# pengfeidip/pytorch-faster-rcnn

Measured on AMD Instinct MI355X. Metric: img/s FasterRCNN_R50_FPN 1000x600 fwd+loss, higher is better.
Workload: dtype f32; 1 GPU; configs/faster_rcnn_r50_fpn.py (BASELINE config 2) forward_train; conv_algorithms=MIOpen benchmarked (warmup, at most 32 tuning iterations per solver), trunk=hipGraph replay (backbone + neck + RPN head convs), global_batch=2, imgs_per_gpu=2, image=600x1000 padded 608x1024, parallelism=dp1, sampler=device, mode=fwd

## Files before the change

pytorch-faster-rcnn_amd/csrc/conv3x3_wino_kernels.h:

```cpp
#pragma once
#include "common.h"

namespace frh {

typedef float wg_f32x16 __attribute__((ext_vector_type(16)));
typedef float wg_f32x2 __attribute__((ext_vector_type(2)));

constexpr int kWgThreads = 256;
constexpr int kWgBK = 8;
constexpr int kWgSide = 8;
constexpr int kWgCout = 64;
constexpr int kWgXcds = 8;
constexpr int kWgMaxLevels = 8;
constexpr int kWgSlab = 64 * kWgBK;
constexpr int kWgStage = 2 * 16 * kWgSlab;

struct Conv3x3Level {
  const float* x;
  const float* u;
  const float* bias;
  float* y;
  int64_t sn;
  int32_t sy, sx;
  int32_t h, w;
  int32_t by, bx;
  int32_t first;
};

struct Conv3x3Args {
  Conv3x3Level lv[kWgMaxLevels];
  int32_t levels, n, cin, cout, relu;
  int32_t total, chunk;
};

__device__ __forceinline__ int wg_slab_off(int r, int kh) { return r * kWgBK + ((kh ^ ((r >> 3) & 1)) << 2); }

struct Conv3x3Weights {
  const float* w[kWgMaxLevels];
  float* u[kWgMaxLevels];
};

__global__ void __launch_bounds__(256) conv3x3_bias_act_weights_kernel(const Conv3x3Weights tab, int cin, int cout) {
  const int64_t idx = (int64_t)blockIdx.x * 256 + threadIdx.x;
  if (idx >= (int64_t)(cin / kWgBK) * cout * 2) return;
  const float* w = tab.w[0];
  float* u = tab.u[0];
#pragma unroll
  for (int i = 1; i < kWgMaxLevels; ++i)
    if (i == (int)blockIdx.y) w = tab.w[i], u = tab.u[i];
  const int kh = (int)(idx & 1);
  const int co = (int)((idx >> 1) % cout);
  const int ch = (int)((idx >> 1) / cout);
  const float* wp = w + (int64_t)co * 9 * cin + ch * kWgBK + kh * 4;
  float g[3][3][4];
#pragma unroll
  for (int ky = 0; ky < 3; ++ky)
#pragma unroll
    for (int kx = 0; kx < 3; ++kx) {
      const float4 v = *reinterpret_cast<const float4*>(wp + (ky * 3 + kx) * cin);
      g[ky][kx][0] = v.x, g[ky][kx][1] = v.y, g[ky][kx][2] = v.z, g[ky][kx][3] = v.w;
    }
  float t[4][3][4];
#pragma unroll
  for (int kx = 0; kx < 3; ++kx)
#pragma unroll
    for (int c = 0; c < 4; ++c) {
      const float s = g[0][kx][c] + g[2][kx][c];
      t[0][kx][c] = g[0][kx][c];
      t[1][kx][c] = (s + g[1][kx][c]) * 0.5f;
      t[2][kx][c] = (s - g[1][kx][c]) * 0.5f;
      t[3][kx][c] = g[2][kx][c];
    }
  float* up = u + ((int64_t)ch * 16 * cout + co) * kWgBK + ((kh ^ ((co >> 3) & 1)) << 2);
#pragma unroll
  for (int a = 0; a < 4; ++a) {
    float o[4][4];
#pragma unroll
    for (int c = 0; c < 4; ++c) {
      const float s = t[a][0][c] + t[a][2][c];
      o[0][c] = t[a][0][c];
      o[1][c] = (s + t[a][1][c]) * 0.5f;
      o[2][c] = (s - t[a][1][c]) * 0.5f;
      o[3][c] = t[a][2][c];
    }
#pragma unroll
    for (int b = 0; b < 4; ++b)
      *reinterpret_cast<float4*>(up + (int64_t)(a * 4 + b) * cout * kWgBK) =
          make_float4(o[b][0], o[b][1], o[b][2], o[b][3]);
  }
}

__global__ void __launch_bounds__(kWgThreads) conv3x3_bias_act_wino_kernel(const Conv3x3Args a) {
  __shared__ __attribute__((aligned(16))) float lds[2 * kWgStage];

  const int wg = (int)(blockIdx.x % kWgXcds) * a.chunk + (int)(blockIdx.x / kWgXcds);
  if (wg >= a.total) return;
  Conv3x3Level L = a.lv[0];
#pragma unroll
  for (int i = 1; i < kWgMaxLevels; ++i)
    if (i < a.levels && wg >= a.lv[i].first) L = a.lv[i];
  const int H = L.h, W = L.w;
  int rest = wg - L.first;
  const int bx = rest % L.bx;
  rest /= L.bx;
  const int by = rest % L.by;
  rest /= L.by;
  const int img = rest % a.n;
  const int cb = rest / a.n;

  const int tid = threadIdx.x;
  const int lane = tid & 63, wave = tid >> 6;
  const int wm = wave >> 1, wn = wave & 1;
  const int h = lane >> 5, j = lane & 31;

  const int T = tid >> 2, c2 = tid & 3;
  const int iy0 = (by * kWgSide + (T >> 3)) * 2 - 1;
  const int ix0 = (bx * kWgSide + (T & 7)) * 2 - 1;
  const char* xb = reinterpret_cast<const char*>(L.x + (int64_t)img * L.sn);
  uint32_t xoff[4][4];
  bool xok[4][4];
#pragma unroll
  for (int r = 0; r < 4; ++r)
#pragma unroll
    for (int c = 0; c < 4; ++c) {
      const int iy = iy0 + r, ix = ix0 + c;
      xok[r][c] = iy >= 0 && iy < H && ix >= 0 && ix < W;
      const int cy = min(max(iy, 0), H - 1), cx = min(max(ix, 0), W - 1);
      xoff[r][c] = (uint32_t)(cy * L.sy + cx * L.sx + c2 * 2) * 4u;
    }
  const int v_off = wg_slab_off(T, c2 >> 1) + (c2 & 1) * 2;
  const char* ub = reinterpret_cast<const char*>(L.u + (int64_t)cb * kWgCout * kWgBK);
  const uint32_t u_src = (uint32_t)((tid >> 7) * a.cout * kWgBK + (tid & 127) * 4) * 4u;
  const int64_t u_pos = (int64_t)2 * a.cout * kWgBK * 4;
  const int64_t u_chunk = (int64_t)16 * a.cout * kWgBK * 4;
  const int u_off = 16 * kWgSlab + (tid >> 7) * kWgSlab + (tid & 127) * 4;
  const int a_off = wg_slab_off(wm * 32 + j, h);
  const int b_off = 16 * kWgSlab + wg_slab_off(wn * 32 + j, h);

  wg_f32x2 x00, x01, x02, x03, x10, x11, x12, x13, x20, x21, x22, x23, x30, x31, x32, x33;
  float4 u0, u1, u2, u3, u4, u5, u6, u7;
#define FRH_WG_LX(r, c) x##r##c = *reinterpret_cast<const wg_f32x2*>(xs_ + xoff[r][c])
#define FRH_WG_LU(q) *reinterpret_cast<const float4*>(up_ + (q) * u_pos + u_src)
#define FRH_WG_LOAD(t)                                                                   \
  do {                                                                                   \
    const char* xs_ = xb + (t) * (kWgBK * 4);                                               \
    FRH_WG_LX(0, 0), FRH_WG_LX(0, 1), FRH_WG_LX(0, 2), FRH_WG_LX(0, 3);                  \
    FRH_WG_LX(1, 0), FRH_WG_LX(1, 1), FRH_WG_LX(1, 2), FRH_WG_LX(1, 3);                  \
    FRH_WG_LX(2, 0), FRH_WG_LX(2, 1), FRH_WG_LX(2, 2), FRH_WG_LX(2, 3);                  \
    FRH_WG_LX(3, 0), FRH_WG_LX(3, 1), FRH_WG_LX(3, 2), FRH_WG_LX(3, 3);                  \
    const char* up_ = ub + (t) * u_chunk;                                                \
    u0 = FRH_WG_LU(0), u1 = FRH_WG_LU(1), u2 = FRH_WG_LU(2), u3 = FRH_WG_LU(3);          \
    u4 = FRH_WG_LU(4), u5 = FRH_WG_LU(5), u6 = FRH_WG_LU(6), u7 = FRH_WG_LU(7);          \
  } while (0)

#define FRH_WG_Z(r, c) (xok[r][c] ? x##r##c : z2)
#define FRH_WG_VROW(vp, e0, e1, e2, e3)                                   \
  do {                                                                    \
    *reinterpret_cast<wg_f32x2*>(vp) = (e0) - (e2);                       \
    *reinterpret_cast<wg_f32x2*>((vp) + kWgSlab) = (e1) + (e2);           \
    *reinterpret_cast<wg_f32x2*>((vp) + 2 * kWgSlab) = (e2) - (e1);       \
    *reinterpret_cast<wg_f32x2*>((vp) + 3 * kWgSlab) = (e1) - (e3);       \
  } while (0)
#define FRH_WG_STORE(ST)                                                                             \
  do {                                                                                               \
    float* sp = lds + (ST) * kWgStage;                                                               \
    float* uq = sp + u_off;                                                                          \
    *reinterpret_cast<float4*>(uq) = u0, *reinterpret_cast<float4*>(uq + 2 * kWgSlab) = u1;          \
    *reinterpret_cast<float4*>(uq + 4 * kWgSlab) = u2, *reinterpret_cast<float4*>(uq + 6 * kWgSlab) = u3;   \
    *reinterpret_cast<float4*>(uq + 8 * kWgSlab) = u4, *reinterpret_cast<float4*>(uq + 10 * kWgSlab) = u5;  \
    *reinterpret_cast<float4*>(uq + 12 * kWgSlab) = u6, *reinterpret_cast<float4*>(uq + 14 * kWgSlab) = u7; \
    const wg_f32x2 z2 = {0.0f, 0.0f};                                                                \
    const wg_f32x2 d00 = FRH_WG_Z(0, 0), d01 = FRH_WG_Z(0, 1), d02 = FRH_WG_Z(0, 2), d03 = FRH_WG_Z(0, 3); \
    const wg_f32x2 d10 = FRH_WG_Z(1, 0), d11 = FRH_WG_Z(1, 1), d12 = FRH_WG_Z(1, 2), d13 = FRH_WG_Z(1, 3); \
    const wg_f32x2 d20 = FRH_WG_Z(2, 0), d21 = FRH_WG_Z(2, 1), d22 = FRH_WG_Z(2, 2), d23 = FRH_WG_Z(2, 3); \
    const wg_f32x2 d30 = FRH_WG_Z(3, 0), d31 = FRH_WG_Z(3, 1), d32 = FRH_WG_Z(3, 2), d33 = FRH_WG_Z(3, 3); \
    float* vp = sp + v_off;                                                                          \
    FRH_WG_VROW(vp, d00 - d20, d01 - d21, d02 - d22, d03 - d23);                                     \
    FRH_WG_VROW(vp + 4 * kWgSlab, d10 + d20, d11 + d21, d12 + d22, d13 + d23);                       \
    FRH_WG_VROW(vp + 8 * kWgSlab, d20 - d10, d21 - d11, d22 - d12, d23 - d13);                       \
    FRH_WG_VROW(vp + 12 * kWgSlab, d10 - d30, d11 - d31, d12 - d32, d13 - d33);                      \
  } while (0)

#define FRH_WG_MFMA(ST, p)                                                          \
  do {                                                                              \
    const float* sp = lds + (ST) * kWgStage + (p) * kWgSlab;                        \
    const float4 av = *reinterpret_cast<const float4*>(sp + a_off);                 \
    const float4 bv = *reinterpret_cast<const float4*>(sp + b_off);                 \
    acc[p] = __builtin_amdgcn_mfma_f32_32x32x2f32(av.x, bv.x, acc[p], 0, 0, 0);     \
    acc[p] = __builtin_amdgcn_mfma_f32_32x32x2f32(av.y, bv.y, acc[p], 0, 0, 0);     \
    acc[p] = __builtin_amdgcn_mfma_f32_32x32x2f32(av.z, bv.z, acc[p], 0, 0, 0);     \
    acc[p] = __builtin_amdgcn_mfma_f32_32x32x2f32(av.w, bv.w, acc[p], 0, 0, 0);     \
  } while (0)

#define FRH_WG_GROUPS(N, MEM, ID)                                                     \
  _Pragma("unroll") for (int p = 0; p < (N); ++p) {                                 \
    __builtin_amdgcn_sched_group_barrier(0x100, 2, ID);                             \
    _Pragma("unroll") for (int m = 0; m < 4; ++m) {                                 \
      __builtin_amdgcn_sched_group_barrier(0x008, 1, ID);                           \
      __builtin_amdgcn_sched_group_barrier(0x002, 2, ID);                           \
      __builtin_amdgcn_sched_group_barrier(MEM, 1, ID);                             \
    }                                                                               \
  }
#define FRH_WG_STEP(ST, STORE, LOAD, t)                                             \
  do {                                                                              \
    _Pragma("unroll") for (int p = 0; p < 16; ++p) FRH_WG_MFMA(ST, p);              \
    if (STORE) FRH_WG_STORE((ST) ^ 1);                                              \
    if (LOAD) FRH_WG_LOAD((t) + 2);                                                 \
    if (STORE) {                                                                    \
      __builtin_amdgcn_sched_group_barrier(0x100, 4, ST);                           \
      FRH_WG_GROUPS(4, 0x200, ST);                                                     \
      FRH_WG_GROUPS(6, 0x020, ST);                                                     \
      FRH_WG_GROUPS(6, 0x200, ST);                                                     \
    }                                                                               \
    if (STORE) {                                                                    \
      __syncthreads();                                                              \
      __builtin_amdgcn_sched_barrier(0);                                            \
    }                                                                               \
  } while (0)

  wg_f32x16 acc[16];
#pragma unroll
  for (int p = 0; p < 16; ++p)
#pragma unroll
    for (int r = 0; r < 16; ++r) acc[p][r] = 0.0f;

  const int steps = a.cin / kWgBK;
  FRH_WG_LOAD(0);
  FRH_WG_STORE(0);
  if (steps > 1) FRH_WG_LOAD(1);
  __syncthreads();
  int t = 0;
  for (; t + 3 < steps; t += 2) {
    FRH_WG_STEP(0, true, true, t);
    FRH_WG_STEP(1, true, true, t + 1);
  }
  if (t + 3 == steps) {
    FRH_WG_STEP(0, true, true, t);
    FRH_WG_STEP(1, true, false, t + 1);
    FRH_WG_STEP(0, false, false, t + 2);
  } else if (t + 2 == steps) {
    FRH_WG_STEP(0, true, false, t);
    FRH_WG_STEP(1, false, false, t + 1);
  } else {
    FRH_WG_STEP(0, false, false, t);
  }
#undef FRH_WG_LX
#undef FRH_WG_LU
#undef FRH_WG_LOAD
#undef FRH_WG_Z
#undef FRH_WG_VROW
#undef FRH_WG_STORE
#undef FRH_WG_MFMA
#undef FRH_WG_GROUPS
#undef FRH_WG_STEP

  const int co = cb * kWgCout + wn * 32 + j;
  const bool has_bias = L.bias != nullptr;
  const float bias = has_bias ? L.bias[co] : 0.0f;
  float* yb = L.y + (int64_t)img * H * W * a.cout + co;
#pragma unroll
  for (int r = 0; r < 16; ++r) {
    const int oy = (by * kWgSide + wm * 4 + (r >> 2)) * 2;
    const int ox = (bx * kWgSide + (r & 3) + 4 * h) * 2;
    float s0[4], s1[4];
#pragma unroll
    for (int b = 0; b < 4; ++b) {
      s0[b] = (acc[b][r] + acc[4 + b][r]) + acc[8 + b][r];
      s1[b] = (acc[4 + b][r] - acc[8 + b][r]) - acc[12 + b][r];
    }
    float o[2][2];
    o[0][0] = (s0[0] + s0[1]) + s0[2];
    o[0][1] = (s0[1] - s0[2]) - s0[3];
    o[1][0] = (s1[0] + s1[1]) + s1[2];
    o[1][1] = (s1[1] - s1[2]) - s1[3];
#pragma unroll
    for (int dy = 0; dy < 2; ++dy)
#pragma unroll
      for (int dx = 0; dx < 2; ++dx) {
        float v = o[dy][dx];
        if (has_bias) v = v + bias;
        if (a.relu) v = fmaxf(v, 0.0f);
        if (oy + dy < H && ox + dx < W) yb[((int64_t)(oy + dy) * W + (ox + dx)) * a.cout] = v;
      }
  }
}

struct Conv3x3LevelDesc {
  const float* x;
  const float* wt;
  const float* bias;
  float* y;
  int32_t h, w;
  int64_t sn, sy, sx;
};

inline int32_t conv3x3_launch(const char* what, int32_t levels, const Conv3x3LevelDesc* d, float* ws,
                              int64_t ws_floats, int64_t n, int32_t cin, int32_t cout, int32_t relu, void* stream) {
  FRH_REQUIRE(levels >= 1 && levels <= kWgMaxLevels, "1 to %d levels, got %d", kWgMaxLevels, levels);
  FRH_REQUIRE(n >= 0 && n < (1 << 20) && cin >= 1 && cout >= 1 && cout <= (1 << 20), "bad sizes");
  FRH_REQUIRE(cin % kWgBK == 0 && cout % kWgCout == 0, "cin %d must be a multiple of %d and cout %d of %d", cin,
              kWgBK, cout, kWgCout);
  FRH_REQUIRE(ws, "null pointer argument");
  FRH_REQUIRE((uintptr_t)ws % 16 == 0, "tensors must be 16-byte aligned");
  const int64_t slot = (int64_t)16 * cin * cout;
  Conv3x3Weights tab = {};
  int slots = 0;
  Conv3x3Args a;
  a.levels = 0, a.n = (int32_t)n, a.cin = cin, a.cout = cout, a.relu = relu;
  int64_t total = 0;
  for (int i = 0; i < levels; ++i) {
    const Conv3x3LevelDesc& s = d[i];
    FRH_REQUIRE(s.h >= 0 && s.w >= 0, "bad sizes");
    if (n == 0 || s.h == 0 || s.w == 0) continue;
    FRH_REQUIRE(s.x && s.y && s.wt, "null pointer argument");
    FRH_REQUIRE(((uintptr_t)s.x | (uintptr_t)s.y | (uintptr_t)s.bias | (uintptr_t)s.wt) % 16 == 0,
                "tensors must be 16-byte aligned");
    if (slots == 0 || tab.w[slots - 1] != s.wt) {
      FRH_REQUIRE((slots + 1) * slot <= ws_floats, "workspace holds %lld floats, %d weights need %lld",
                  (long long)ws_floats, slots + 1, (long long)((slots + 1) * slot));
      tab.w[slots] = s.wt, tab.u[slots] = ws + slots * slot;
      ++slots;
    }
    FRH_REQUIRE(s.sn >= 0 && s.sy >= 0 && s.sx >= cin && (s.sn | s.sy | s.sx) % 4 == 0,
                "x strides must be multiples of 4 elements and the column stride at least cin");
    const int64_t span = (int64_t)(s.h - 1) * s.sy + (int64_t)(s.w - 1) * s.sx + cin;
    FRH_REQUIRE(span < ((int64_t)1 << 30), "one image of x spans too many elements");
    const int64_t x_end = (n - 1) * s.sn + span, y_end = n * s.h * s.w * cout;
    FRH_REQUIRE(s.y + y_end <= s.x || s.x + x_end <= s.y, "y must not alias x");
    FRH_REQUIRE(s.y + y_end <= ws || ws + ws_floats <= s.y, "y must not alias the workspace");
    Conv3x3Level& L = a.lv[a.levels++];
    L.x = s.x, L.u = tab.u[slots - 1], L.bias = s.bias, L.y = s.y;
    L.sn = s.sn, L.sy = (int32_t)s.sy, L.sx = (int32_t)s.sx, L.h = s.h, L.w = s.w;
    L.by = (s.h + 2 * kWgSide - 1) / (2 * kWgSide), L.bx = (s.w + 2 * kWgSide - 1) / (2 * kWgSide);
    L.first = (int32_t)total;
    total += (int64_t)L.by * L.bx * n * (cout / kWgCout);
    FRH_REQUIRE(total < ((int64_t)1 << 30), "too many blocks");
  }
  if (a.levels == 0) return FRH_OK;
  a.total = (int32_t)total;
  a.chunk = (int32_t)((total + kWgXcds - 1) / kWgXcds);
  const int64_t wt = (int64_t)(cin / kWgBK) * cout * 2;
  hipLaunchKernelGGL(conv3x3_bias_act_weights_kernel, dim3((unsigned)((wt + 255) / 256), (unsigned)slots), dim3(256),
                     0, as_stream(stream), tab, cin, cout);
  hipLaunchKernelGGL(conv3x3_bias_act_wino_kernel, dim3((unsigned)(a.chunk * kWgXcds)), dim3(kWgThreads), 0,
                     as_stream(stream), a);
  return check_launch(what);
}

}
```

Before: 376.0 img/s.

## Stream Winograd filter tiles via direct global-to-LDS loads and buffer loads

The Winograd 3x3 conv kernel now copies filter tiles straight from global memory into LDS with global_load_lds_dwordx4 through inline asm, instead of loading them into registers and storing them to LDS. Input tiles are read with raw buffer loads, which makes out-of-range reads safe, and are double-buffered in registers two steps ahead. The main loop is simplified to clamped step indices, with a combined waitcnt and barrier and a retuned schedule-group interleave. This is meant to cut VGPR pressure and VALU/LDS-store work in the main loop. In exchange it relies on hand-written m0 handling in inline asm and does redundant loads on the final steps.

```diff
diff --git a/pytorch-faster-rcnn_amd/csrc/conv3x3_wino_kernels.h b/pytorch-faster-rcnn_amd/csrc/conv3x3_wino_kernels.h
--- a/pytorch-faster-rcnn_amd/csrc/conv3x3_wino_kernels.h
+++ b/pytorch-faster-rcnn_amd/csrc/conv3x3_wino_kernels.h
@@ -13,7 +13,10 @@
 constexpr int kWgXcds = 8;
 constexpr int kWgMaxLevels = 8;
 constexpr int kWgSlab = 64 * kWgBK;
-constexpr int kWgStage = 2 * 16 * kWgSlab;
+constexpr int kWgImage = 16 * kWgSlab;
+
+typedef uint32_t wg_u32x2 __attribute__((ext_vector_type(2)));
+typedef __attribute__((address_space(3))) void* wg_lds_ptr;
 
 struct Conv3x3Level {
   const float* x;
@@ -90,8 +93,22 @@
   }
 }
 
+__device__ __forceinline__ __amdgpu_buffer_rsrc_t wg_buffer(const void* p) {
+  const uint64_t v = reinterpret_cast<uint64_t>(p);
+  const uint32_t lo = __builtin_amdgcn_readfirstlane((uint32_t)v);
+  const uint32_t hi = __builtin_amdgcn_readfirstlane((uint32_t)(v >> 32));
+  return __builtin_amdgcn_make_buffer_rsrc(reinterpret_cast<void*>(((uint64_t)hi << 32) | lo), 0, -1, 0x00020000);
+}
+
+__device__ __forceinline__ uint64_t wg_uniform64(const void* p) {
+  const uint64_t v = reinterpret_cast<uint64_t>(p);
+  const uint32_t lo = __builtin_amdgcn_readfirstlane((uint32_t)v);
+  const uint32_t hi = __builtin_amdgcn_readfirstlane((uint32_t)(v >> 32));
+  return ((uint64_t)hi << 32) | lo;
+}
+
 __global__ void __launch_bounds__(kWgThreads) conv3x3_bias_act_wino_kernel(const Conv3x3Args a) {
-  __shared__ __attribute__((aligned(16))) float lds[2 * kWgStage];
+  __shared__ __attribute__((aligned(16))) float lds[4 * kWgImage];
 
   const int wg = (int)(blockIdx.x % kWgXcds) * a.chunk + (int)(blockIdx.x / kWgXcds);
   if (wg >= a.total) return;
@@ -109,14 +126,14 @@
   const int cb = rest / a.n;
 
   const int tid = threadIdx.x;
-  const int lane = tid & 63, wave = tid >> 6;
+  const int lane = tid & 63, wave = __builtin_amdgcn_readfirstlane(tid >> 6);
   const int wm = wave >> 1, wn = wave & 1;
   const int h = lane >> 5, j = lane & 31;
 
   const int T = tid >> 2, c2 = tid & 3;
   const int iy0 = (by * kWgSide + (T >> 3)) * 2 - 1;
   const int ix0 = (bx * kWgSide + (T & 7)) * 2 - 1;
-  const char* xb = reinterpret_cast<const char*>(L.x + (int64_t)img * L.sn);
+  const __amdgpu_buffer_rsrc_t xb = wg_buffer(L.x + (int64_t)img * L.sn);
   uint32_t xoff[4][4];
   bool xok[4][4];
 #pragma unroll
@@ -129,31 +146,51 @@
       xoff[r][c] = (uint32_t)(cy * L.sy + cx * L.sx + c2 * 2) * 4u;
     }
   const int v_off = wg_slab_off(T, c2 >> 1) + (c2 & 1) * 2;
-  const char* ub = reinterpret_cast<const char*>(L.u + (int64_t)cb * kWgCout * kWgBK);
-  const uint32_t u_src = (uint32_t)((tid >> 7) * a.cout * kWgBK + (tid & 127) * 4) * 4u;
-  const int64_t u_pos = (int64_t)2 * a.cout * kWgBK * 4;
-  const int64_t u_chunk = (int64_t)16 * a.cout * kWgBK * 4;
-  const int u_off = 16 * kWgSlab + (tid >> 7) * kWgSlab + (tid & 127) * 4;
-  const int a_off = wg_slab_off(wm * 32 + j, h);
-  const int b_off = 16 * kWgSlab + wg_slab_off(wn * 32 + j, h);
-
-  wg_f32x2 x00, x01, x02, x03, x10, x11, x12, x13, x20, x21, x22, x23, x30, x31, x32, x33;
-  float4 u0, u1, u2, u3, u4, u5, u6, u7;
-#define FRH_WG_LX(r, c) x##r##c = *reinterpret_cast<const wg_f32x2*>(xs_ + xoff[r][c])
-#define FRH_WG_LU(q) *reinterpret_cast<const float4*>(up_ + (q) * u_pos + u_src)
-#define FRH_WG_LOAD(t)                                                                   \
-  do {                                                                                   \
-    const char* xs_ = xb + (t) * (kWgBK * 4);                                               \
-    FRH_WG_LX(0, 0), FRH_WG_LX(0, 1), FRH_WG_LX(0, 2), FRH_WG_LX(0, 3);                  \
-    FRH_WG_LX(1, 0), FRH_WG_LX(1, 1), FRH_WG_LX(1, 2), FRH_WG_LX(1, 3);                  \
-    FRH_WG_LX(2, 0), FRH_WG_LX(2, 1), FRH_WG_LX(2, 2), FRH_WG_LX(2, 3);                  \
-    FRH_WG_LX(3, 0), FRH_WG_LX(3, 1), FRH_WG_LX(3, 2), FRH_WG_LX(3, 3);                  \
-    const char* up_ = ub + (t) * u_chunk;                                                \
-    u0 = FRH_WG_LU(0), u1 = FRH_WG_LU(1), u2 = FRH_WG_LU(2), u3 = FRH_WG_LU(3);          \
-    u4 = FRH_WG_LU(4), u5 = FRH_WG_LU(5), u6 = FRH_WG_LU(6), u7 = FRH_WG_LU(7);          \
-  } while (0)
-
-#define FRH_WG_Z(r, c) (xok[r][c] ? x##r##c : z2)
+  const int64_t u_pos = (int64_t)a.cout * kWgBK * 4;
+  const int64_t u_chunk = 16 * u_pos;
+  const char* ub = reinterpret_cast<const char*>(L.u + (int64_t)cb * kWgCout * kWgBK) + wave * 4 * u_pos;
+  const uint32_t u_lane = (uint32_t)lane * 16u;
+  const uint32_t u_dst = (uint32_t)(uintptr_t)(wg_lds_ptr)lds + (uint32_t)wave * 4 * kWgSlab * 4;
+  const int a_off = 2 * kWgImage + wg_slab_off(wm * 32 + j, h);
+  const int b_off = wg_slab_off(wn * 32 + j, h);
+
+  wg_f32x2 x000, x001, x002, x003, x010, x011, x012, x013, x020, x021, x022, x023, x030, x031, x032, x033;
+  wg_f32x2 x100, x101, x102, x103, x110, x111, x112, x113, x120, x121, x122, x123, x130, x131, x132, x133;
+  const wg_f32x2 z2 = {0.0f, 0.0f};
+#define FRH_WG_LX(S, r, c) \
+  x##S##r##c = __builtin_bit_cast(wg_f32x2, __builtin_amdgcn_raw_buffer_load_b64(xb, (int)xoff[r][c], xs_, 0))
+#define FRH_WG_LOADX(S, t)                                                                       \
+  do {                                                                                           \
+    const int xs_ = (t) * (kWgBK * 4);                                                           \
+    FRH_WG_LX(S, 0, 0), FRH_WG_LX(S, 0, 1), FRH_WG_LX(S, 0, 2), FRH_WG_LX(S, 0, 3);              \
+    FRH_WG_LX(S, 1, 0), FRH_WG_LX(S, 1, 1), FRH_WG_LX(S, 1, 2), FRH_WG_LX(S, 1, 3);              \
+    FRH_WG_LX(S, 2, 0), FRH_WG_LX(S, 2, 1), FRH_WG_LX(S, 2, 2), FRH_WG_LX(S, 2, 3);              \
+    FRH_WG_LX(S, 3, 0), FRH_WG_LX(S, 3, 1), FRH_WG_LX(S, 3, 2), FRH_WG_LX(S, 3, 3);              \
+  } while (0)
+
+#define FRH_WG_DMA(ST, t, after)                                                                 \
+  do {                                                                                           \
+    const uint64_t g_ = wg_uniform64(ub + (int64_t)(t) * u_chunk);                               \
+    const uint32_t l_ = u_dst + (ST) * kWgImage * 4;                                             \
+    uint32_t m0_;                                                                                \
+    asm("s_nop 4\n\t"                                                                            \
+        "s_mov_b32 %0, m0\n\t"                                                                   \
+        "s_mov_b32 m0, %3\n\ts_nop 0\n\t"                                                        \
+        "global_load_lds_dwordx4 %2, %7\n\tglobal_load_lds_dwordx4 %2, %7 offset:1024\n\t"       \
+        "s_mov_b32 m0, %4\n\ts_nop 0\n\t"                                                        \
+        "global_load_lds_dwordx4 %2, %8\n\tglobal_load_lds_dwordx4 %2, %8 offset:1024\n\t"       \
+        "s_mov_b32 m0, %5\n\ts_nop 0\n\t"                                                        \
+        "global_load_lds_dwordx4 %2, %9\n\tglobal_load_lds_dwordx4 %2, %9 offset:1024\n\t"       \
+        "s_mov_b32 m0, %6\n\ts_nop 0\n\t"                                                        \
+        "global_load_lds_dwordx4 %2, %10\n\tglobal_load_lds_dwordx4 %2, %10 offset:1024\n\t"     \
+        "s_mov_b32 m0, %0"                                                                       \
+        : "=&s"(m0_), "+v"(token)                                                                \
+        : "v"(u_lane), "s"(l_), "s"(l_ + kWgSlab * 4), "s"(l_ + 2 * kWgSlab * 4),                \
+          "s"(l_ + 3 * kWgSlab * 4), "s"(g_), "s"(g_ + u_pos), "s"(g_ + 2 * u_pos),              \
+          "s"(g_ + 3 * u_pos), "v"(after));                                                      \
+  } while (0)
+
+#define FRH_WG_Z(S, r, c) (xok[r][c] ? x##S##r##c : z2)
 #define FRH_WG_VROW(vp, e0, e1, e2, e3)                                   \
   do {                                                                    \
     *reinterpret_cast<wg_f32x2*>(vp) = (e0) - (e2);                       \
@@ -161,29 +198,22 @@
     *reinterpret_cast<wg_f32x2*>((vp) + 2 * kWgSlab) = (e2) - (e1);       \
     *reinterpret_cast<wg_f32x2*>((vp) + 3 * kWgSlab) = (e1) - (e3);       \
   } while (0)
-#define FRH_WG_STORE(ST)                                                                             \
-  do {                                                                                               \
-    float* sp = lds + (ST) * kWgStage;                                                               \
-    float* uq = sp + u_off;                                                                          \
-    *reinterpret_cast<float4*>(uq) = u0, *reinterpret_cast<float4*>(uq + 2 * kWgSlab) = u1;          \
-    *reinterpret_cast<float4*>(uq + 4 * kWgSlab) = u2, *reinterpret_cast<float4*>(uq + 6 * kWgSlab) = u3;   \
-    *reinterpret_cast<float4*>(uq + 8 * kWgSlab) = u4, *reinterpret_cast<float4*>(uq + 10 * kWgSlab) = u5;  \
-    *reinterpret_cast<float4*>(uq + 12 * kWgSlab) = u6, *reinterpret_cast<float4*>(uq + 14 * kWgSlab) = u7; \
-    const wg_f32x2 z2 = {0.0f, 0.0f};                                                                \
-    const wg_f32x2 d00 = FRH_WG_Z(0, 0), d01 = FRH_WG_Z(0, 1), d02 = FRH_WG_Z(0, 2), d03 = FRH_WG_Z(0, 3); \
-    const wg_f32x2 d10 = FRH_WG_Z(1, 0), d11 = FRH_WG_Z(1, 1), d12 = FRH_WG_Z(1, 2), d13 = FRH_WG_Z(1, 3); \
-    const wg_f32x2 d20 = FRH_WG_Z(2, 0), d21 = FRH_WG_Z(2, 1), d22 = FRH_WG_Z(2, 2), d23 = FRH_WG_Z(2, 3); \
-    const wg_f32x2 d30 = FRH_WG_Z(3, 0), d31 = FRH_WG_Z(3, 1), d32 = FRH_WG_Z(3, 2), d33 = FRH_WG_Z(3, 3); \
-    float* vp = sp + v_off;                                                                          \
-    FRH_WG_VROW(vp, d00 - d20, d01 - d21, d02 - d22, d03 - d23);                                     \
-    FRH_WG_VROW(vp + 4 * kWgSlab, d10 + d20, d11 + d21, d12 + d22, d13 + d23);                       \
-    FRH_WG_VROW(vp + 8 * kWgSlab, d20 - d10, d21 - d11, d22 - d12, d23 - d13);                       \
-    FRH_WG_VROW(vp + 12 * kWgSlab, d10 - d30, d11 - d31, d12 - d32, d13 - d33);                      \
+#define FRH_WG_VSTORE(ST, S)                                                                               \
+  do {                                                                                                     \
+    const wg_f32x2 d00 = FRH_WG_Z(S, 0, 0), d01 = FRH_WG_Z(S, 0, 1), d02 = FRH_WG_Z(S, 0, 2), d03 = FRH_WG_Z(S, 0, 3); \
+    const wg_f32x2 d10 = FRH_WG_Z(S, 1, 0), d11 = FRH_WG_Z(S, 1, 1), d12 = FRH_WG_Z(S, 1, 2), d13 = FRH_WG_Z(S, 1, 3); \
+    const wg_f32x2 d20 = FRH_WG_Z(S, 2, 0), d21 = FRH_WG_Z(S, 2, 1), d22 = FRH_WG_Z(S, 2, 2), d23 = FRH_WG_Z(S, 2, 3); \
+    const wg_f32x2 d30 = FRH_WG_Z(S, 3, 0), d31 = FRH_WG_Z(S, 3, 1), d32 = FRH_WG_Z(S, 3, 2), d33 = FRH_WG_Z(S, 3, 3); \
+    float* vp = lds + (2 + (ST)) * kWgImage + v_off;                                                       \
+    FRH_WG_VROW(vp, d00 - d20, d01 - d21, d02 - d22, d03 - d23);                                           \
+    FRH_WG_VROW(vp + 4 * kWgSlab, d10 + d20, d11 + d21, d12 + d22, d13 + d23);                             \
+    FRH_WG_VROW(vp + 8 * kWgSlab, d20 - d10, d21 - d11, d22 - d12, d23 - d13);                             \
+    FRH_WG_VROW(vp + 12 * kWgSlab, d10 - d30, d11 - d31, d12 - d32, d13 - d33);                            \
   } while (0)
 
 #define FRH_WG_MFMA(ST, p)                                                          \
   do {                                                                              \
-    const float* sp = lds + (ST) * kWgStage + (p) * kWgSlab;                        \
+    const float* sp = lds + (ST) * kWgImage + (p) * kWgSlab;                        \
     const float4 av = *reinterpret_cast<const float4*>(sp + a_off);                 \
     const float4 bv = *reinterpret_cast<const float4*>(sp + b_off);                 \
     acc[p] = __builtin_amdgcn_mfma_f32_32x32x2f32(av.x, bv.x, acc[p], 0, 0, 0);     \
@@ -192,30 +222,31 @@
     acc[p] = __builtin_amdgcn_mfma_f32_32x32x2f32(av.w, bv.w, acc[p], 0, 0, 0);     \
   } while (0)
 
-#define FRH_WG_GROUPS(N, MEM, ID)                                                     \
+#define FRH_WG_SYNC()                                                                        \
+  do {                                                                                       \
+    asm volatile("s_waitcnt vmcnt(0) lgkmcnt(0)\n\ts_barrier" : "+v"(token) : : "memory");    \
+    __builtin_amdgcn_sched_barrier(0);                                                       \
+  } while (0)
+
+#define FRH_WG_GROUPS(N, VALU, MEM, K, ID)                                          \
   _Pragma("unroll") for (int p = 0; p < (N); ++p) {                                 \
     __builtin_amdgcn_sched_group_barrier(0x100, 2, ID);                             \
     _Pragma("unroll") for (int m = 0; m < 4; ++m) {                                 \
       __builtin_amdgcn_sched_group_barrier(0x008, 1, ID);                           \
-      __builtin_amdgcn_sched_group_barrier(0x002, 2, ID);                           \
-      __builtin_amdgcn_sched_group_barrier(MEM, 1, ID);                             \
+      __builtin_amdgcn_sched_group_barrier(0x002, VALU, ID);                        \
+      __builtin_amdgcn_sched_group_barrier(MEM, K, ID);                             \
     }                                                                               \
   }
-#define FRH_WG_STEP(ST, STORE, LOAD, t)                                             \
+#define FRH_WG_STEP(ST, OT, t)                                                        \
   do {                                                                              \
     _Pragma("unroll") for (int p = 0; p < 16; ++p) FRH_WG_MFMA(ST, p);              \
-    if (STORE) FRH_WG_STORE((ST) ^ 1);                                              \
-    if (LOAD) FRH_WG_LOAD((t) + 2);                                                 \
-    if (STORE) {                                                                    \
-      __builtin_amdgcn_sched_group_barrier(0x100, 4, ST);                           \
-      FRH_WG_GROUPS(4, 0x200, ST);                                                     \
-      FRH_WG_GROUPS(6, 0x020, ST);                                                     \
-      FRH_WG_GROUPS(6, 0x200, ST);                                                     \
-    }                                                                               \
-    if (STORE) {                                                                    \
-      __syncthreads();                                                              \
-      __builtin_amdgcn_sched_barrier(0);                                            \
-    }                                                                               \
+    FRH_WG_LOADX(ST, min((t) + 2, last));                                           \
+    FRH_WG_DMA(OT, min((t) + 1, last), FRH_WG_Z(OT, 3, 3).y);                       \
+    FRH_WG_VSTORE(OT, OT);                                                          \
+    __builtin_amdgcn_sched_group_barrier(0x100, 4, ST);                             \
+    FRH_WG_GROUPS(2, 4, 0x020, 2, ST);                                              \
+    FRH_WG_GROUPS(14, 2, 0x200, 1, ST);                                             \
+    FRH_WG_SYNC();                                                                  \
   } while (0)
 
   wg_f32x16 acc[16];
@@ -224,33 +255,27 @@
 #pragma unroll
     for (int r = 0; r < 16; ++r) acc[p][r] = 0.0f;
 
-  const int steps = a.cin / kWgBK;
-  FRH_WG_LOAD(0);
-  FRH_WG_STORE(0);
-  if (steps > 1) FRH_WG_LOAD(1);
-  __syncthreads();
-  int t = 0;
-  for (; t + 3 < steps; t += 2) {
-    FRH_WG_STEP(0, true, true, t);
-    FRH_WG_STEP(1, true, true, t + 1);
-  }
-  if (t + 3 == steps) {
-    FRH_WG_STEP(0, true, true, t);
-    FRH_WG_STEP(1, true, false, t + 1);
-    FRH_WG_STEP(0, false, false, t + 2);
-  } else if (t + 2 == steps) {
-    FRH_WG_STEP(0, true, false, t);
-    FRH_WG_STEP(1, false, false, t + 1);
-  } else {
-    FRH_WG_STEP(0, false, false, t);
+  const int last = a.cin / kWgBK - 1;
+  uint32_t token = 0;
+  FRH_WG_DMA(0, 0, 0.0f);
+  FRH_WG_LOADX(0, 0);
+  FRH_WG_LOADX(1, min(1, last));
+  FRH_WG_VSTORE(0, 0);
+  FRH_WG_SYNC();
+  for (int t = 0;; t += 2) {
+    FRH_WG_STEP(0, 1, t);
+    if (t >= last) break;
+    FRH_WG_STEP(1, 0, t + 1);
+    if (t + 1 >= last) break;
   }
 #undef FRH_WG_LX
-#undef FRH_WG_LU
-#undef FRH_WG_LOAD
+#undef FRH_WG_LOADX
+#undef FRH_WG_DMA
 #undef FRH_WG_Z
 #undef FRH_WG_VROW
-#undef FRH_WG_STORE
+#undef FRH_WG_VSTORE
 #undef FRH_WG_MFMA
+#undef FRH_WG_SYNC
 #undef FRH_WG_GROUPS
 #undef FRH_WG_STEP
 
```

Measured after the change: 398.8 img/s (median of 6 runs). 6.1% higher.
